# openai/iaf

Measured on AMD Instinct MI355X. Metric: IAF-step samples/sec (down_iaf2_nl posterior stack, forward + log-det), higher is better.
Workload: dtype f32 (operands split into 2 fp16 planes hi + lo 2^-11, 3 part-products on the fp16 MFMA in two fp32 accumulators: fp32-grade error, operands up to 65504)

## Files before the change

### iaf_amd/csrc/iaf_step_fused.hpp

```cpp
#pragma once
#include "iaf_conv_bf3.hpp"
#include "iaf_step_fused_types.hpp"
#ifndef IAF_HELPER_PRIO
#define IAF_HELPER_PRIO 0
#endif

#ifndef IAF_EXP_HOUT
#define IAF_EXP_HOUT 1
#endif
#ifndef IAF_EXP_HOUT8
#define IAF_EXP_HOUT8 1
#endif
template <int NHT, int NZT, int DEPTH, int W, int R, int XCH = 0, int PAIR = 0, int F16 = 0>
struct StepGeom {
    static constexpr int NZ = 16 * NZT, NH = 16 * NHT;
    static constexpr int NPL = F16 ? 2 : 3;
    static constexpr int RS = W + 2;
    static constexpr int Z8 = NZ / 8, Z16 = NPL * Z8 + 2;
    static constexpr int H8 = NH / 8, H16 = NPL * H8 + 2;
    static constexpr int RZ = XCH ? R + 1 : R + DEPTH + 1;
    static constexpr int rows_h(int l) { return XCH ? R : R + DEPTH - l; }
    static constexpr int rows_reg(int l) { return XCH ? R + 1 : R + DEPTH - l; }
    static constexpr int ZREG = 0;
    static constexpr int HREG0 = ZREG + RZ * RS * Z16;
// ... 250 lines not shown
    constexpr int CPX = G::CPX, CSTR = G::CSTR, CG = CPX / 4, NCIT = NH * CG, NCI = (NCIT + 255) / 256;
    f32x4 cv[NCI], cv2[NCI];
    unsigned cvalid = 0;
    auto load_ctx = [&]() {
        const int vpx = (H - r0) * W < CPX ? (H - r0) * W : CPX;
        constexpr bool REG = (256 % CG == 0) && (NCIT % 256 == 0);
        unsigned gi0 = 0, gstep = 0;
        bool in0 = true;
        if constexpr (REG) {
            const int c = tid / CG, g4 = (tid - c * CG) * 4;
            in0 = g4 < vpx;
            const int g4c = in0 ? g4 : 0;
            const int row = g4c / W, col4 = g4c - row * W;
            gi0 = 4u * (unsigned)(c * HW + gpix(r0 + row, col4 + (FLIP ? 3 : 0)));
            gstep = 4u * (unsigned)((256 / CG) * HW);
        }
        auto ctx_off = [&](int u, bool& inside) -> unsigned {
            if constexpr (REG) { inside = in0; return gi0 + (unsigned)u * gstep; }
            const int idx = tid + u * 256;
            const int ic = idx < NCIT ? idx : NCIT - 1;
            const int c = ic / CG, g4 = (ic - c * CG) * 4;
            inside = g4 < vpx;
            const int g4c = inside ? g4 : 0;
            const int row = g4c / W, col4 = g4c - row * W;
            return 4u * (unsigned)(c * HW + gpix(r0 + row, col4 + (FLIP ? 3 : 0)));
        };
#pragma unroll
        for (int u = 0; u < NCI; ++u) {
            bool inside;
            const unsigned gi = ctx_off(u, inside);
            cv[u] = ldf4(p.ctx + img_h, gi);
            cvalid |= (inside ? 1u : 0u) << u;
        }
        if (p.ctx2) {
#pragma unroll
            for (int u = 0; u < NCI; ++u) {
                bool inside;
                const unsigned gi = ctx_off(u, inside);
                cv2[u] = ldf4(p.ctx2 + img_h, gi);
            }
        }
    };
    auto zero_cols = [&]() {
        constexpr int ZROWS = RZ, H0ROWS = G::rows_reg(0), H1ROWS = 0;
        for (int i = tid; i < ZROWS * 2 * Z16; i += 256) {
            const int rs = i / Z16, u = i - rs * Z16;
            smem4[G::ZREG + ((rs >> 1) * RS + (rs & 1) * (W + 1)) * Z16 + u] = f32x4{0.f, 0.f, 0.f, 0.f};
        }
        for (int i = tid; i < (H0ROWS + H1ROWS) * 2 * H16; i += 256) {
            const int rs = i / H16, u = i - rs * H16;
            const int row = rs >> 1;
            const int base = row < H0ROWS ? G::HREG0 + row * RS * H16 : G::HREG1 + (row - H0ROWS) * RS * H16;
            smem4[base + (rs & 1) * (W + 1) * H16 + u] = f32x4{0.f, 0.f, 0.f, 0.f};
        }
    };
    auto stage_z = [&]() {
#pragma unroll
        for (int u = 0; u < ZU; ++u) {
            const int idx = tid + u * 256;
            if (idx < NIT) {
                const int q = idx / NPX, px = idx - q * NPX;
                const int row = px / W, col = px - row * W;
                f32x4 v = zv[u];
                if (!p.z) {
#pragma unroll
                    for (int r = 0; r < 4; ++r)
                        v[r] = (zv[u][r] + zq[0][u][r]) + __expf(0.5f * (2.f * (zq[1][u][r] + zq[2][u][r]))) * zq[3][u][r];
                }
                if (r0 + row >= H) v = f32x4{0.f, 0.f, 0.f, 0.f};
                split_store4(smem + (size_t)G::ZREG * 16, row * RS + col + 1, q, v, Z16, Z8);
            }
        }
    };

    constexpr unsigned XNLST = IAF_XCTL_LISTS;
    unsigned xcc = 0, xdead = 0;
    unsigned long long xdone = 0, xlists_done = 0;
    [[maybe_unused]] unsigned xmine = 0, xmine_n = 0;
    int xslot = 0;
    int half = 0;
    [[maybe_unused]] unsigned long long xt0 = 0;
    [[maybe_unused]] unsigned xlist = 0, xnl = 1;
    unsigned* xmail = (unsigned*)(smem + (size_t)G::CTX_OFF * 16);
    auto xch_take_begin = [&]() {
        if constexpr (TKT) {
            if (tid == 0) {
                asm volatile("s_getreg_b32 %0, hwreg(HW_REG_XCC_ID, 0, 4)" : "=s"(xcc));
                xcc &= 7u;
                xlist = xcc & (XNLST - 1u);
                if (p.xknob & 1u) xlist = (blockIdx.x * 2654435761u >> 13) & (XNLST - 1u);
                xnl = (unsigned)p.B < XNLST ? (unsigned)p.B : XNLST;
                if (xnl < XNLST) xlist %= xnl;
                if (p.xknob & 2u)
                    for (unsigned i = 0, n = (blockIdx.x * 40503u >> 4) & 63u; i < n; ++i) __builtin_amdgcn_s_sleep(64);
                xt0 = __hip_atomic_fetch_add(p.xctl + 32 * xlist, 1ull, __ATOMIC_RELAXED, XSCOPE);
                xdead = (unsigned)__hip_atomic_load(p.xctl + IAF_XCTL_STICKY, __ATOMIC_RELAXED, XSCOPE);
            }
        }
    };
    auto xch_take_finish = [&]() {
        if constexpr (TKT) {
            if (tid == 0) {
                unsigned long long v = xt0;
                unsigned y = xlist, t = 0, ny = 0;
                bool found = false;
                for (unsigned k = 0; k < xnl; ++k) {
                    if (k) { y = (xlist + k) % xnl; v = __hip_atomic_fetch_add(p.xctl + 32 * y, 1ull, __ATOMIC_RELAXED, XSCOPE); }
                    ny = (int)y < p.B ? (PAIR ? 2u : 1u) * (unsigned)p.nrb * (unsigned)((p.B - (int)y + (int)XNLST - 1) / (int)XNLST) : 0u;
                    t = (unsigned)v;
                    if (t < ny) { found = true; break; }
                }
                xmine = y; xmine_n = found ? ny : 0u;
                if (found) xdone = __hip_atomic_fetch_add(p.xctl + 32 * y + 16, 1ull, __ATOMIC_RELAXED, XSCOPE);
                unsigned ib = 0, ir = (unsigned)p.nrb - 1;
                const unsigned ti = PAIR ? t >> 1 : t;
                if (found) { ib = y + XNLST * (ti / (unsigned)p.nrb); ir = (unsigned)p.nrb - 1u - ti % (unsigned)p.nrb; }
                else xdead |= 2u;
                xmail[0] = ib; xmail[1] = ir; xmail[2] = xdead; xmail[3] = t & 1u;
                if (p.dbg) p.dbg[(size_t)blockIdx.x * 32 + 30] = 1ull + (((unsigned long long)y << 32) | t);
            }
            __syncthreads();
            b = __builtin_amdgcn_readfirstlane((int)xmail[0]);
            rbk = __builtin_amdgcn_readfirstlane((int)xmail[1]);
            xdead = __builtin_amdgcn_readfirstlane(xmail[2]);
            if constexpr (PAIR) half = __builtin_amdgcn_readfirstlane((int)xmail[3]);
            r0 = rbk * R;
            img_z = (size_t)b * NZ * HW; img_h = (size_t)b * NH * HW;
            xslot = b * p.nrb + rbk;
            if (xdead && tid == 0) {
                if (p.xerr) __hip_atomic_store(p.xerr, 0x100u | xdead, __ATOMIC_RELAXED, __HIP_MEMORY_SCOPE_SYSTEM);
                __hip_atomic_store(p.xctl + IAF_XCTL_STICKY, (unsigned long long)xdead, __ATOMIC_RELAXED, XSCOPE);
            }
        }
    };
    auto xch_next_epoch_a = [&]() {
        if constexpr (TKT) {
            if (tid == 0 && xmine_n && (unsigned)xdone == xmine_n - 1u)
                xlists_done = __hip_atomic_fetch_add(p.xctl + IAF_XCTL_DONE, 1ull, __ATOMIC_RELAXED, XSCOPE) + 1ull;
        }
    };
    auto xch_next_epoch_b = [&]() {
        if constexpr (TKT) {
            if (tid == 0 && (unsigned)xlists_done == (unsigned)(p.B < (int)XNLST ? p.B : (int)XNLST)) {
                for (int y = 0; y < (int)XNLST; ++y) {
                    __hip_atomic_store(p.xctl + 32 * y, 0ull, __ATOMIC_RELAXED, XSCOPE);
                    __hip_atomic_store(p.xctl + 32 * y + 16, 0ull, __ATOMIC_RELAXED, XSCOPE);
                }
                __hip_atomic_store(p.xctl + IAF_XCTL_DONE, 0ull, __ATOMIC_RELAXED, XSCOPE);
            }
        }
    };

    if constexpr (TKT) {
        xch_take_begin();
        if (!is_helper) {
            preload_w0();
            zero_cols();
        }
        xch_take_finish();
        if (!is_helper) {
            load_z();
            __builtin_amdgcn_sched_barrier(0);
            IAF_FSTAMP(8);
            stage_z();
        }
    } else if (!is_helper) {
        load_z();
        __builtin_amdgcn_sched_barrier(0);
        preload_w0();
        __builtin_amdgcn_sched_barrier(0);
        if constexpr (!HELP) load_ctx();
        __builtin_amdgcn_sched_barrier(0);
        IAF_FSTAMP(8);
        zero_cols();
        stage_z();
    }
    IAF_FSTAMP(9);
    __syncthreads();
    IAF_FSTAMP(1);
    auto store_ctx = [&]() {
        float* creg = (float*)(smem + (size_t)G::CTX_OFF * 16);
#pragma unroll
        for (int u = 0; u < NCI; ++u) {
            const int idx = tid + u * 256;
            if (NCIT % 256 == 0 || idx < NCIT) {
                const int c = idx / CG, g4 = (idx - c * CG) * 4;
                constexpr bool fl = FLIP;
                f32x4 v = cv[u];
                if (p.ctx2) v += cv2[u];
                if (!((cvalid >> u) & 1u)) v = f32x4{0.f, 0.f, 0.f, 0.f};
                *(f32x4*)(creg + c * CSTR + g4) = f32x4{fl ? v[3] : v[0], fl ? v[2] : v[1], fl ? v[1] : v[2], fl ? v[0] : v[3]};
            }
        }
    };

    int qbase = 0;
    auto conv_phase = [&](auto rd_c, auto npt_c, auto ntw_c, auto rows_c, auto emask_c, int in_reg, int in_s16, int in_c8, const f32x4* wbase,
                          int ncot, const int* tiles, f32x4 (*wr)[decltype(ntw_c)::value][3],
                          f32x4 (*acc_out)[decltype(ntw_c)::value], auto part_c, auto grp_c, auto accum_c, int pair0) __attribute__((always_inline)) {
        typedef decltype(part_c) P;
        constexpr int NPT = decltype(npt_c)::value, NTW = decltype(ntw_c)::value, ROWS = decltype(rows_c)::value;
        constexpr bool TRI = P::TAIL != 0;
        constexpr int nstep = P::NSTEP, s0 = 0;
        constexpr int EMASK = decltype(emask_c)::value;
        constexpr int LALLV = (EMASK == 0 && NTW > 1) ? ((1 << (NTW - 1)) - 1) : -1;
        constexpr std::integral_constant<int, LALLV> LALL{};
        constexpr int RD = decltype(rd_c)::value, U = RD + 1;
        constexpr int GRP = decltype(grp_c)::value;
        constexpr bool TALL = GRP >= 300 && GRP < 400, PTRI = GRP >= 100 && GRP < 300, HCMP = GRP >= 400;
        constexpr int PSG = F16 ? (NTW >= 2 ? 2 : 3) : TALL ? 1 : fused_acc_groups(HCMP ? NTWH : NTW);
        f32x4 acc[PSG][NPT][NTW];
        int xb[NPT];
#pragma unroll
        for (int q = 0; q < NPT; ++q) {
            int pix = (q + qbase) * 16 + pl;
            pix = pix < ROWS * W ? pix : ROWS * W - 1;
            const int row = pix / W, col = pix - row * W;
            xb[q] = in_reg + (row * RS + col + 1) * in_s16 + kk;
#pragma unroll
            for (int g = 0; g < PSG; ++g)
#pragma unroll
                for (int j = 0; j < NTW; ++j) acc[g][q][j] = f32x4{0.f, 0.f, 0.f, 0.f};
        }
        auto xaddr = [&](auto q_c, int s) __attribute__((always_inline)) -> int {
            int pair, tap;
            P::at(s < nstep ? s : nstep - 1, pair, tap);
// ... 164 lines not shown
                        const int pix = (q + qbase) * 16 + pl;
                        const int row = pix / W, col = pix - row * W;
                        if (pix < ROWS * W && row < R && r0 + row < H && (!save_half || (htile[j] >= NHT / 2) == (half != 0)))
                            *(f32x4*)(hsave + ((size_t)b * HW + (size_t)gpix(r0 + row, col)) * NH + htile[j] * 16 + 4 * kk) = vout[j][q];
                    }
                });
            }
            return;
        }
#pragma unroll
        for (int oi = 0; oi < NTWH * NPT; ++oi) {
            const int j = oi / NPT, q = oi % NPT;
            if (htile[j] >= NHT) continue;
            const f32x4 bi = bias[j];
            {
                if (j == NTWH - 1 && !((EMASK >> q) & 1)) continue;
                const int pix = (q + qbase) * 16 + pl;
                if (pix >= ROWS * W) continue;
                const int row = pix / W, col = pix - row * W;
                f32x4 v = acc[q][j] + bi;
                if constexpr (BORDER) { if (r0 + row < H) v += border_terms(bt, NH, htile[j] * 16 + 4 * kk, r0 + row, col); }
                if constexpr (WITH_CTX) v += cxv[q][j];
#pragma unroll
                for (int r = 0; r < 4; ++r) v[r] = elu_f(v[r]);
                if (r0 + row >= H) v = f32x4{0.f, 0.f, 0.f, 0.f};
                split_store4(smem + (size_t)out_reg * 16, row * RS + col + 1, htile[j] * 4 + kk, v, H16, H8);
                if (hsave && row < R && r0 + row < H && (!save_half || (htile[j] >= NHT / 2) == (half != 0)))
                    *(f32x4*)(hsave + ((size_t)b * HW + (size_t)gpix(r0 + row, col)) * NH + htile[j] * 16 + 4 * kk) = v;
            }
        }
    };

    constexpr int NZF = PAIR ? NZ / 2 : NZ;
    constexpr int NEL = (NZF * R * W + 255) / 256;
    float fz[NEL], fq[NEL][6];
    float fb[NEL][2];
    auto load_final_operands = [&]() {
        const int fcb = PAIR ? half * NZF : 0;
#pragma unroll
        for (int e = 0; e < NEL; ++e) {
            const int idx = tid + e * 256;
            const int ic = idx < NZF * R * W ? idx : NZF * R * W - 1;
            const int c = fcb + ic / (R * W), pix = ic % (R * W);
            const int rr = r0 + pix / W < H ? r0 + pix / W : H - 1;
            const unsigned gi = 4u * (unsigned)(c * HW + gpix(rr, pix & (W - 1)));
            const int cm = (c >> 4) * 32 + (c & 15);
            fb[e][0] = p.bias[DEPTH][cm]; fb[e][1] = p.bias[DEPTH][cm + 16];
            fz[e] = 0.f;
            if (p.mode == MODE_IAF || p.mode == MODE_INVERSE) fz[e] = ldf(p.zin + img_z, gi);
            if (p.mode == MODE_POSTERIOR) {
                fq[e][0] = ldf(p.qm + img_z, gi) + ldf(p.rm + img_z, gi); fq[e][1] = ldf(p.ql + img_z, gi) + ldf(p.rl + img_z, gi);
                fq[e][2] = ldf(p.eps + img_z, gi); fq[e][3] = ldf(p.pm + img_z, gi); fq[e][4] = ldf(p.pl + img_z, gi);
            }
        }
    };
    constexpr unsigned XSENT = F16 ? IAF_XSENT_F16 : IAF_XSENT;
    constexpr unsigned XNAN = F16 ? 0x7e007e00u : 0x7fc07fc0u;
    constexpr int XSC1 = 16;
    constexpr int XNU = W * H16, XNL = (XNU + 255) / 256;
    auto xch_rsrc = [&](int l, int slot) -> __amdgpu_buffer_rsrc_t {
        const unsigned long long a = (unsigned long long)(p.xh + ((size_t)l * p.B * p.nrb + slot) * G::xrow_bytes());
        const unsigned lo = __builtin_amdgcn_readfirstlane((unsigned)a), hi = __builtin_amdgcn_readfirstlane((unsigned)(a >> 32));
        return __builtin_amdgcn_make_buffer_rsrc((void*)(((unsigned long long)hi << 32) | lo), 0, (int)G::xrow_bytes(), 0x00020000);
    };
    constexpr int XNLH = (XNU + 255) / 256;
    auto xch_export = [&](int l, int reg) {
        if constexpr (XCH) {
            if (rbk > 0 && !((p.xknob & 8u) && b == 0 && rbk == p.nrb - 1 && l == 0)) {
                const __amdgpu_buffer_rsrc_t r = xch_rsrc(l, xslot);
                const f32x4* src = smem4 + reg + H16;
                f32x4 t[XNLH];
#pragma unroll
                for (int u = 0; u < XNLH; ++u) { const int i = htid + 256 * u; t[u] = src[i < XNU ? i : XNU - 1]; }
#pragma unroll
                for (int u = 0; u < XNLH; ++u)
                    __builtin_amdgcn_raw_buffer_store_b128(__builtin_bit_cast(u32x4, t[u]), r, 16 * (htid + 256 * u), 0, XSC1);
                if (l == 0 && p.dbg && htid == 0) {
                    p.dbg[(size_t)blockIdx.x * 32 + 27] = __builtin_readcyclecounter();
                    p.dbg[(size_t)blockIdx.x * 32 + 26] = (unsigned long long)xslot + 1;
                }
            }
        }
    };
    auto xch_import = [&](int l, int reg) {
        if constexpr (XCH) {
            f32x4* dst = smem4 + reg + (R * RS + 1) * H16;
            if (r0 + R < H) {
                const __amdgpu_buffer_rsrc_t r = xch_rsrc(l, xslot + 1);
                u32x4 t[XNLH];
                unsigned pad = 0;
#pragma unroll
                for (int u = 0; u < XNLH; ++u) {
                    const int i = htid + 256 * u;
                    if (i >= XNU || (i % H16) >= NPL * H8) pad |= 1u << u;
                }
                const int tmo = (p.xknob & 8u) ? (1 << 10) : (1 << 20);
                int it = xdead ? tmo : 0;
                if (p.dbg && htid == 0) p.dbg[(size_t)blockIdx.x * 32 + (l == 0 ? 14 : 18)] = __builtin_readcyclecounter();
                while (it < tmo) {
                    bool ok = true;
#pragma unroll
                    for (int u = 0; u < XNLH; ++u) t[u] = __builtin_amdgcn_raw_buffer_load_b128(r, 16 * (htid + 256 * u), 0, XSC1);
#pragma unroll
                    for (int u = 0; u < XNLH; ++u)
                        ok = ok && (((pad >> u) & 1u) || (t[u][0] != XSENT && t[u][1] != XSENT && t[u][2] != XSENT && t[u][3] != XSENT));
                    if (__all(ok)) break;
                    __builtin_amdgcn_s_sleep(8);
                    ++it;
                }
                if (p.dbg && htid == 0) {
                    p.dbg[(size_t)blockIdx.x * 32 + (l == 0 ? 16 : 19)] = __builtin_readcyclecounter();
                    p.dbg[(size_t)blockIdx.x * 32 + (l == 0 ? 24 : 25)] = (unsigned long long)it + 1;
                    p.dbg[(size_t)blockIdx.x * 32 + 26] = (unsigned long long)xslot + 1;
                }
                if (it < tmo) {
#pragma unroll
                    for (int u = 0; u < XNLH; ++u)
                        __builtin_amdgcn_raw_buffer_store_b128(u32x4{XSENT, XSENT, XSENT, XSENT}, r, 16 * (htid + 256 * u), 0, XSC1);
                } else {
#pragma unroll
                    for (int u = 0; u < XNLH; ++u) t[u] = u32x4{XNAN, XNAN, XNAN, XNAN};
                    if (lane == 0 && !xdead) {
                        if (p.xerr) __hip_atomic_store(p.xerr, 1u, __ATOMIC_RELAXED, __HIP_MEMORY_SCOPE_SYSTEM);
                        __hip_atomic_store(p.xctl + IAF_XCTL_STICKY, 1ull, __ATOMIC_RELAXED, XSCOPE);
                    }
                }
#pragma unroll
                for (int u = 0; u < XNLH; ++u) { const int i = htid + 256 * u; if (i < XNU) dst[i] = __builtin_bit_cast(f32x4, t[u]); }
                if (p.dbg && htid == 0) p.dbg[(size_t)blockIdx.x * 32 + (l == 0 ? 17 : 20)] = __builtin_readcyclecounter();
            } else {
                for (int i = htid; i < XNU; i += 256) dst[i] = f32x4{0.f, 0.f, 0.f, 0.f};
            }
        }
    };
    constexpr int PNL = PAIR ? (G::PUNITS + 255) / 256 : 1;
    constexpr int LASTH = ((DEPTH - 1) & 1) ? G::HREG1 : G::HREG0;
    auto pair_rsrc = [&](int hf) -> __amdgpu_buffer_rsrc_t {
        const unsigned long long a = (unsigned long long)(p.xh + ((size_t)xslot * 2 + hf) * G::prow_bytes());
        const unsigned lo = __builtin_amdgcn_readfirstlane((unsigned)a), hi = __builtin_amdgcn_readfirstlane((unsigned)(a >> 32));
        return __builtin_amdgcn_make_buffer_rsrc((void*)(((unsigned long long)hi << 32) | lo), 0, (int)G::prow_bytes(), 0x00020000);
    };
    auto pair_lds = [&](int i, int hf) -> int {
        const int sl = i / G::PUS, rem = i - sl * G::PUS;
        const int pn = rem / (H8 / 2), u = rem - pn * (H8 / 2);
        const int row = sl / W, col = sl - row * W;
        return LASTH + (row * RS + col + 1) * H16 + pn * H8 + hf * (H8 / 2) + u;
    };
    auto pair_export = [&]() {
        if constexpr (PAIR) {
            const __amdgpu_buffer_rsrc_t r = pair_rsrc(half);
            u32x4 t[PNL];
#pragma unroll
            for (int u = 0; u < PNL; ++u) {
                const int i = htid + 256 * u;
                t[u] = __builtin_bit_cast(u32x4, smem4[pair_lds(i < G::PUNITS ? i : G::PUNITS - 1, half)]);
            }
#pragma unroll
            for (int u = 0; u < PNL; ++u)
                __builtin_amdgcn_raw_buffer_store_b128(t[u], r, 16 * (htid + 256 * u), 0, XSC1);
            if (p.dbg && htid == 0) p.dbg[(size_t)blockIdx.x * 32 + 27] = __builtin_readcyclecounter();
        }
    };
    auto pair_import = [&]() {
        if constexpr (PAIR) {
            const __amdgpu_buffer_rsrc_t r = pair_rsrc(half ^ 1);
            u32x4 t[PNL];
            unsigned pad = 0;
#pragma unroll
            for (int u = 0; u < PNL; ++u)
                if (htid + 256 * u >= G::PUNITS) pad |= 1u << u;
            const int tmo = (p.xknob & 8u) ? (1 << 10) : (1 << 20);
            int it = xdead ? tmo : 0;
            if (p.dbg && htid == 0) p.dbg[(size_t)blockIdx.x * 32 + 18] = __builtin_readcyclecounter();
            while (it < tmo) {
                bool ok = true;
#pragma unroll
                for (int u = 0; u < PNL; ++u) t[u] = __builtin_amdgcn_raw_buffer_load_b128(r, 16 * (htid + 256 * u), 0, XSC1);
#pragma unroll
                for (int u = 0; u < PNL; ++u)
                    ok = ok && (((pad >> u) & 1u) || (t[u][0] != XSENT && t[u][1] != XSENT && t[u][2] != XSENT && t[u][3] != XSENT));
                if (__all(ok)) break;
                __builtin_amdgcn_s_sleep(8);
                ++it;
            }
            if (p.dbg && htid == 0) {
                p.dbg[(size_t)blockIdx.x * 32 + 19] = __builtin_readcyclecounter();
                p.dbg[(size_t)blockIdx.x * 32 + 25] = (unsigned long long)it + 1;
                p.dbg[(size_t)blockIdx.x * 32 + 26] = (unsigned long long)(2 * xslot + half) + 1;
            }
            const bool taken = it < tmo;
            if (!taken) {
#pragma unroll
                for (int u = 0; u < PNL; ++u) t[u] = u32x4{XNAN, XNAN, XNAN, XNAN};
            }
#pragma unroll
            for (int u = 0; u < PNL; ++u) { const int i = htid + 256 * u; if (i < G::PUNITS) smem4[pair_lds(i, half ^ 1)] = __builtin_bit_cast(f32x4, t[u]); }
            asm volatile("s_waitcnt lgkmcnt(0)" ::: "memory");
            __builtin_amdgcn_s_barrier();
            if (p.dbg && htid == 0) p.dbg[(size_t)blockIdx.x * 32 + 20] = __builtin_readcyclecounter();
            if (taken) {
#pragma unroll
                for (int u = 0; u < PNL; ++u)
                    __builtin_amdgcn_raw_buffer_store_b128(u32x4{XSENT, XSENT, XSENT, XSENT}, r, 16 * (htid + 256 * u), 0, XSC1);
            } else if (lane == 0 && !xdead) {
                if (p.xerr) __hip_atomic_store(p.xerr, 1u, __ATOMIC_RELAXED, __HIP_MEMORY_SCOPE_SYSTEM);
                __hip_atomic_store(p.xctl + IAF_XCTL_STICKY, 1ull, __ATOMIC_RELAXED, XSCOPE);
            }
        }
    };
    if constexpr (HELP) {
        if (is_helper) {
            __builtin_amdgcn_s_setprio(IAF_HELPER_PRIO);
            {
                constexpr int NCIH = (NCIT + 255) / 256;
                float* creg = (float*)(smem + (size_t)G::CTX_OFF * 16);
                const int vpx = (H - r0) * W < CPX ? (H - r0) * W : CPX;
                constexpr int RDL0 = PartL0::NSTEP - 1;
                [[maybe_unused]] f32x4 accu0[1][1], biu0[1], wrl0[HL0 ? RDL0 + 1 : 1][1][3];
                [[maybe_unused]] int lt0[1] = {NW * NFULL + (wave - NW_COMPUTE) % (NX ? NX : 1)};
                [[maybe_unused]] int q0 = -1;
                if constexpr (HL0) {
                    static_for<GN>([&](auto g_c) {
                        constexpr int GI = decltype(g_c)::value;
                        constexpr int EM = fused_extra_mask(NPT0, GN, GI);
                        static_assert(fused_popcount(EM) <= 1, "HL0: one pixel tile per left-over unit");
                        if constexpr (EM != 0) {
                            if ((wave - NW_COMPUTE) / NX == GI) q0 = EM == 1 ? 0 : EM == 2 ? 1 : EM == 4 ? 2 : 3;
                        }
                    });
                }
                f32x4 v[NCIH], v2[NCIH];
                unsigned cval = 0;
#pragma unroll
                for (int u = 0; u < NCIH; ++u) {
                    const int idx = htid + 256 * u, ic = idx < NCIT ? idx : NCIT - 1;
                    const int c = ic / CG, g4 = (ic - c * CG) * 4;
                    const bool inside = g4 < vpx;
                    const int g4c = inside ? g4 : 0, row = g4c / W, col4 = g4c - row * W;
                    const unsigned gi = 4u * (unsigned)(c * HW + gpix(r0 + row, col4 + (FLIP ? 3 : 0)));
                    v[u] = ldf4(p.ctx + img_h, gi);
                    if (p.ctx2) v2[u] = ldf4(p.ctx2 + img_h, gi);
                    cval |= (inside ? 1u : 0u) << u;
                }
                if constexpr (HL0) {
                    if (q0 >= 0) {
                        static_for<RDL0>([&](auto i) {
                            ring_load(std::integral_constant<int, 0>{}, std::integral_constant<int, NPL>{}, wrl0[decltype(i)::value], wb0, NHT, lt0,
                                      PartL0{}, decltype(i)::value, std::integral_constant<int, -1>{}, 0);
                        });
                        load_bias(std::integral_constant<int, 1>{}, lt0, p.bias[0], biu0);
                        qbase = q0;
                        conv_phase(std::integral_constant<int, RDL0>{}, std::integral_constant<int, 1>{}, std::integral_constant<int, 1>{},
                                   std::integral_constant<int, G::rows_h(0)>{}, std::integral_constant<int, 1>{}, G::ZREG, Z16, Z8, wb0, NHT, lt0,
                                   wrl0, accu0, PartL0{}, std::integral_constant<int, 300>{}, std::integral_constant<bool, false>{}, 0);
                        qbase = 0;
                    }
                }
#pragma unroll
                for (int u = 0; u < NCIH; ++u) {
                    const int idx = htid + 256 * u;
                    if (idx < NCIT) {
                        const int c = idx / CG, g4 = (idx - c * CG) * 4;
                        f32x4 t = v[u];
                        if (p.ctx2) t += v2[u];
                        if (!((cval >> u) & 1u)) t = f32x4{0.f, 0.f, 0.f, 0.f};
                        *(f32x4*)(creg + c * CSTR + g4) = FLIP ? f32x4{t[3], t[2], t[1], t[0]} : t;
                    }
                }
                __syncthreads();
                if constexpr (HL0) {
                    if (q0 >= 0) {
                        qbase = q0;
                        hidden_epilogue(std::integral_constant<int, 1>{}, std::integral_constant<int, G::rows_h(0)>{}, std::integral_constant<int, 1>{},
                                        std::integral_constant<int, 1>{}, std::integral_constant<int, 1>{}, lt0, accu0, biu0, G::HREG0, p.hsave[0],
                                        p.border[0], false);
                        qbase = 0;
                    }
                }
            }
            __syncthreads();
            xch_export(0, G::HREG0);
            typedef PairPart<NH / 32, 1> PartO8H;
            constexpr int RDOH8 = 3;
            [[maybe_unused]] f32x4 wroh8[G::HOUT8 ? RDOH8 + 1 : 1][NTWO][3];
            [[maybe_unused]] int ot8[NTWO];
#pragma unroll
            for (int j = 0; j < NTWO; ++j) ot8[j] = (wave - NW_COMPUTE) * NTWO + j;
            static_for<DEPTH - 1>([&](auto lm_c) {
                constexpr int l = decltype(lm_c)::value + 1;
                constexpr int IN_REG = ((l - 1) & 1) ? G::HREG1 : G::HREG0, OUT_REG = (l & 1) ? G::HREG1 : G::HREG0;
                if constexpr (XCH) {
                    xch_import(l - 1, IN_REG);
                    __syncthreads();
                }
                if constexpr (HLEFT) {
                    const int hw = wave - NW_COMPUTE;
                    constexpr int NPTL = (G::rows_h(l) * W + 15) / 16;
                    static_for<GN>([&](auto g_c) {
                        constexpr int GI = decltype(g_c)::value;
                        constexpr int EM = fused_extra_mask(NPTL, GN, GI);
                        static_assert(fused_popcount(EM) <= 1, "HLEFT: one pixel tile per left-over unit");
                        if constexpr (EM != 0) {
                            if (hw / NX != GI) return;
                            int lt[1] = {NW * NFULL + hw % NX};
                            qbase = EM == 1 ? 0 : EM == 2 ? 1 : EM == 4 ? 2 : 3;
                            const f32x4* wbl = (const f32x4*)p.wp3[l];
                            constexpr int RDL = 6;
                            f32x4 wrl[RDL + 1][1][3], accu[1][1], biu[1];
                            static_for<RDL>([&](auto i) {
                                ring_load(std::integral_constant<int, 0>{}, std::integral_constant<int, NPL>{}, wrl[decltype(i)::value], wbl, NHT, lt,
                                          PartHid{}, decltype(i)::value, std::integral_constant<int, -1>{}, 0);
                            });
                            load_bias(std::integral_constant<int, 1>{}, lt, p.bias[l], biu);
                            conv_phase(std::integral_constant<int, RDL>{}, std::integral_constant<int, 1>{}, std::integral_constant<int, 1>{},
                                       std::integral_constant<int, G::rows_h(l)>{}, std::integral_constant<int, 1>{}, IN_REG, H16, H8, wbl, NHT, lt,
                                       wrl, accu, PartHid{}, std::integral_constant<int, 300>{}, std::integral_constant<bool, false>{}, 0);
                            hidden_epilogue(std::integral_constant<int, 1>{}, std::integral_constant<int, G::rows_h(l)>{},
                                            std::integral_constant<int, 1>{}, std::integral_constant<int, 0>{}, std::integral_constant<int, 1>{}, lt,
                                            accu, biu, OUT_REG, p.hsave[l], p.border[l], false);
                            qbase = 0;
                        }
                    });
                }
                if constexpr (G::HOUT8 && l == DEPTH - 1) {
                    static_for<RDOH8>([&](auto i) {
                        ring_load(std::integral_constant<int, 0>{}, std::integral_constant<int, NTWO * NPL>{}, wroh8[decltype(i)::value],
                                  (const f32x4*)p.wp3[DEPTH], 2 * NZT, ot8, PartO8H{}, decltype(i)::value, std::integral_constant<int, -1>{}, 0);
                    });
                }
                __syncthreads();
                xch_export(l, OUT_REG);
            });
            if constexpr (XCH) {
                constexpr int LAST_REG = ((DEPTH - 1) & 1) ? G::HREG1 : G::HREG0;
                xch_import(DEPTH - 1, LAST_REG);
                if constexpr (G::HOUT) {
                    constexpr int NPTO_ = (R * W + 15) / 16;
                    const int hw = wave - NW_COMPUTE;
                    int ot[NTWO];
#pragma unroll
                    for (int j = 0; j < NTWO; ++j) ot[j] = hw * NTWO + j;
                    typedef BelowPar<NH / 32, 1> PartOBH;
                    constexpr int RDOH = 3;
                    const f32x4* wboh = (const f32x4*)p.wp3[DEPTH];
                    f32x4 wroh[RDOH + 1][NTWO][3], accoh[NPTO_][NTWO];
                    static_for<RDOH>([&](auto i) {
                        ring_load(std::integral_constant<int, 0>{}, std::integral_constant<int, NTWO * NPL>{}, wroh[decltype(i)::value], wboh, 2 * NZT,
                                  ot, PartOBH{}, decltype(i)::value, std::integral_constant<int, -1>{}, 0);
                    });
                    __syncthreads();
                    conv_phase(std::integral_constant<int, RDOH>{}, std::integral_constant<int, NPTO_>{}, std::integral_constant<int, NTWO>{},
                               std::integral_constant<int, R>{}, std::integral_constant<int, (1 << NPTO_) - 1>{}, LAST_REG,
                               H16, H8, wboh, 2 * NZT, ot, wroh, accoh, PartOBH{}, std::integral_constant<int, 0>{},
                               std::integral_constant<bool, false>{}, 0);
                    float* part1 = (float*)(smem + (size_t)G::XB_OFF * 16) + R * W * G::XB_STRIDE;
#pragma unroll
                    for (int j = 0; j < NTWO; ++j)
#pragma unroll
                        for (int q = 0; q < NPTO_; ++q) {
                            const int pix = q * 16 + pl;
                            if (pix >= R * W) continue;
#pragma unroll
                            for (int r = 0; r < 4; ++r) part1[pix * G::XB_STRIDE + ot[j] * 16 + 4 * kk + r] = accoh[q][j][r];
                        }
                } else {
                    __syncthreads();
                }
            }
            if constexpr (PAIR) {
                if (!((p.xknob & 8u) && b == 0 && rbk == 0 && half == 1)) pair_export();
                pair_import();
            }
            if constexpr (G::HOUT8) {
                constexpr int NPTO_ = (R * W + 15) / 16, LAST_REG = ((DEPTH - 1) & 1) ? G::HREG1 : G::HREG0;
                const f32x4* wboh = (const f32x4*)p.wp3[DEPTH];
                f32x4 accoh[NPTO_][NTWO];
                conv_phase(std::integral_constant<int, RDOH8>{}, std::integral_constant<int, NPTO_>{}, std::integral_constant<int, NTWO>{},
                           std::integral_constant<int, R>{}, std::integral_constant<int, (1 << NPTO_) - 1>{}, LAST_REG,
                           H16, H8, wboh, 2 * NZT, ot8, wroh8, accoh, PartO8H{}, std::integral_constant<int, 0>{},
                           std::integral_constant<bool, false>{}, 0);
                float* part1 = (float*)(smem + (size_t)G::XB_OFF * 16) + R * W * G::XB_STRIDE;
#pragma unroll
                for (int j = 0; j < NTWO; ++j)
#pragma unroll
                    for (int q = 0; q < NPTO_; ++q) {
                        const int pix = q * 16 + pl;
                        if (pix >= R * W) continue;
#pragma unroll
                        for (int r = 0; r < 4; ++r) part1[pix * G::XB_STRIDE + ot8[j] * 16 + 4 * kk + r] = accoh[q][j][r];
                    }
            }
            raise_range();
            __syncthreads();
            if (p.fin_ctl && p.mode == MODE_POSTERIOR) {
                unsigned* fmail = (unsigned*)smem;
                __syncthreads();
                if (htid == 0) {
                    const unsigned g = blockIdx.x & 7u, ng = (gridDim.x - g + 7u) >> 3, ngroups = gridDim.x < 8u ? gridDim.x : 8u;
                    unsigned last = 0;
                    if ((unsigned)__hip_atomic_fetch_add(p.fin_ctl + 32 * g, 1ull, __ATOMIC_RELAXED, XSCOPE) == ng - 1u) {
                        __hip_atomic_store(p.fin_ctl + 32 * g, 0ull, __ATOMIC_RELAXED, XSCOPE);
                        if ((unsigned)__hip_atomic_fetch_add(p.fin_ctl + 256, 1ull, __ATOMIC_RELAXED, XSCOPE) == ngroups - 1u) {
                            __hip_atomic_store(p.fin_ctl + 256, 0ull, __ATOMIC_RELAXED, XSCOPE);
                            last = 1;
                        }
                    }
                    fmail[0] = last;
                }
                __syncthreads();
                if (!fmail[0]) return;
                float* S = (float*)smem + 64;
                {
                    const __amdgpu_buffer_rsrc_t r = __builtin_amdgcn_make_buffer_rsrc((void*)p.kl_part, 0, p.B * p.nrb * NZ * 4, 0x00020000);
                    constexpr int Z4 = NZ / 4;
                    for (int i = htid; i < p.B * Z4; i += 256) {
                        const int bb = i / Z4, c4 = i - bb * Z4;
                        f32x4 a = f32x4{0.f, 0.f, 0.f, 0.f};
                        for (int k0 = 0; k0 < p.nrb; k0 += 8) {
                            u32x4 v8[8];
#pragma unroll
                            for (int k = 0; k < 8; ++k) {
                                const int rr = k0 + k < p.nrb ? k0 + k : p.nrb - 1;
                                v8[k] = __builtin_amdgcn_raw_buffer_load_b128(r, 4 * ((bb * p.nrb + rr) * NZ + 4 * c4), 0, XSC1);
                            }
#pragma unroll
                            for (int k = 0; k < 8; ++k)
                                if (k0 + k < p.nrb) a += __builtin_bit_cast(f32x4, v8[k]);
                        }
                        *(f32x4*)(S + (size_t)bb * NZ + 4 * c4) = a;
                    }
                }
                __syncthreads();
                if (htid < 64) {
                    const int GR = p.B / p.fin_groups;
                    float fbv = 0.f;
                    for (int g = 0; g < p.fin_groups; ++g) {
                        float a = 0.f;
                        if (htid < NZ) {
                            const float* Sg = S + (size_t)g * GR * NZ;
                            float m = 0.f;
                            for (int bb = 0; bb < GR; ++bb) m += Sg[(size_t)bb * NZ + htid];
                            a = fmaxf(m / (float)GR, p.fin_kl_min);
                            if (p.fin_gate && p.fin_kl_min > 0.f) p.fin_gate[g * NZ + htid] = (m / (float)GR > p.fin_kl_min) ? 1.f : 0.f;
                        }
#pragma unroll
                        for (int o = 32; o > 0; o >>= 1) a += __shfl_down(a, o, 64);
                        const float fb = __shfl(a, 0, 64);
                        if (htid == g) fbv = fb;
                    }
                    for (int b0 = 0; b0 < p.B; b0 += 64) {
// ... 11 lines not shown
            return;
        }
    }

    typedef std::conditional_t<XCH != 0, std::conditional_t<VAR == 0, PartOwnTri, PartOwn>, PartHid> PartH1;
    constexpr bool HO8 = G::HOUT8 && HELP;
    constexpr bool XK2 = PAIR || G::HOUT || HO8;
    typedef std::conditional_t<XCH != 0, PartOwn, std::conditional_t<HO8, PairPart<NPAIR_H, 0>, PartFull>> PartO1;
    int otile[NTWO];
#pragma unroll
    for (int j = 0; j < NTWO; ++j) otile[j] = wave * NTWO + j;
    constexpr int NHTP = NHT / 2, NFULLP = NHTP / NW, NTWP = NFULLP + 1;
    int ptile[NTWP];
    f32x4 wrp[PAIR ? UB : 1][NTWP][3];
    if constexpr (PAIR) {
#pragma unroll
        for (int j = 0; j < NTWP; ++j)
            ptile[j] = NHTP * half + ((j < NFULLP) ? ((j & 1) ? NW * (j + 1) - 1 - wave : wave + NW * j) : NW * NFULLP);
    }
    const int opar = wave & 1;
    constexpr int NPO = (NH / 2) / 32, NPR = NPAIR_H - NPO;
    const int opair_own = half ? NPAIR_H - NPO : 0, opair_rest = half ? 0 : NPO;
    if constexpr (PAIR) otile[0] = NZT * half + (wave >> 1);
    f32x4 wr1[UB][NTWH][3];
    f32x4 wrh1[HLEFT ? UB : 1][NTW1][3];
    f32x4 wro[UO][NTWO][3];
    const f32x4* wbo = (const f32x4*)p.wp3[DEPTH];
    auto preload_out = [&]() __attribute__((always_inline)) {
        if constexpr (PAIR) {
            static_for<2>([&](auto par_c) {
                if (opar != decltype(par_c)::value) return;
                static_for<RDO>([&](auto i) {
                    ring_load(std::integral_constant<int, 0>{}, std::integral_constant<int, NTWO * NPL>{}, wro[decltype(i)::value], wbo, 2 * NZT,
                              otile, PairPart<NPO, decltype(par_c)::value>{}, decltype(i)::value, ALL, opair_own);
                });
            });
            return;
        }
        static_for<RDO>([&](auto i) {
            ring_load(std::integral_constant<int, 0>{}, std::integral_constant<int, NTWO * NPL>{}, wro[decltype(i)::value], wbo, 2 * NZT,
                      otile, PartO1{}, decltype(i)::value, ALL, 0);
        });
    };
    auto preload_after = [&](auto l_c) __attribute__((always_inline)) {
        constexpr int l = decltype(l_c)::value;
        if constexpr (PAIR && l + 1 < DEPTH) {
            const f32x4* wbn = (const f32x4*)p.wp3[l + 1];
            static_for<RDH>([&](auto i) {
                ring_load(std::integral_constant<int, 0>{}, std::integral_constant<int, NTWP * NPL>{}, wrp[decltype(i)::value], wbn, NHT, ptile,
                          PartHid{}, decltype(i)::value, ALL, 0);
            });
        } else if constexpr (l + 1 < DEPTH && HLEFT) {
            const f32x4* wbn = (const f32x4*)p.wp3[l + 1];
            static_for<RDH>([&](auto i) {
                ring_load(std::integral_constant<int, 0>{}, std::integral_constant<int, NTW1 * NPL>{}, wrh1[decltype(i)::value], wbn, NHT, htile,
                          PartH1{}, decltype(i)::value, ALL, 0);
            });
        } else if constexpr (l + 1 < DEPTH) {
            const f32x4* wbn = (const f32x4*)p.wp3[l + 1];
            static_for<RDH>([&](auto i) {
                ring_load(std::integral_constant<int, 0>{}, std::integral_constant<int, NTWH * NPL>{},
                          ((l + 1) & 1) ? wr1[decltype(i)::value] : wr0[decltype(i)::value], wbn, NHT, htile, PartH1{}, decltype(i)::value,
                          ALL, 0);
            });
        } else {
            preload_out();
        }
    };
    static_for<GN>([&](auto g_c) {
        constexpr int GI = decltype(g_c)::value;
        if (xg != GI) return;
        constexpr int EM0 = HL0 ? (1 << NPT0) - 1 : (NX == 0 || !XSPLIT) ? (1 << NPT0) - 1 : fused_extra_mask(NPT0, GN, GI);
        f32x4 acc0[NPT0][NTW0], bi0[NTW0];
        load_bias(std::integral_constant<int, NTW0>{}, htile, p.bias[0], bi0);
        if constexpr (HL0)
            conv_phase(std::integral_constant<int, RD0>{}, std::integral_constant<int, NPT0>{}, std::integral_constant<int, NTW0>{},
                       std::integral_constant<int, G::rows_h(0)>{}, std::integral_constant<int, EM0>{}, G::ZREG, Z16, Z8, wb0, NHT, htile,
                       wrh0, acc0, PartL0{}, std::integral_constant<int, 400 + GI>{}, SET, 0);
        else
            conv_phase(std::integral_constant<int, RD0>{}, std::integral_constant<int, NPT0>{}, std::integral_constant<int, NTW0>{},
                       std::integral_constant<int, G::rows_h(0)>{}, std::integral_constant<int, EM0>{}, G::ZREG, Z16, Z8, wb0, NHT, htile,
                       wr0, acc0, PartL0{}, g_c, SET, 0);
        IAF_FSTAMP(6);
        xch_next_epoch_a();
        if constexpr (!HELP) store_ctx();
        if constexpr (DEPTH == 1) load_final_operands();
        preload_after(std::integral_constant<int, 0>{});
        IAF_FSTAMP(10);
        __syncthreads();
        IAF_FSTAMP(11);
        hidden_epilogue(std::integral_constant<int, NPT0>{}, std::integral_constant<int, G::rows_h(0)>{},
                        std::integral_constant<int, EM0>{}, std::integral_constant<int, 1>{}, std::integral_constant<int, NTW0>{}, htile, acc0, bi0,
                        G::HREG0, p.hsave[0], p.border[0], PAIR != 0);
    });
    __syncthreads();
    IAF_FSTAMP(2);
    if constexpr (PAIR) {
        constexpr int l = 1, IN_REG = G::HREG0, OUT_REG = G::HREG1;
        {
            constexpr int H1ROWS = G::rows_reg(1);
            for (int i = tid; i < H1ROWS * 2 * H16; i += 256) {
                const int rs = i / H16, u = i - rs * H16;
                smem4[G::HREG1 + ((rs >> 1) * RS + (rs & 1) * (W + 1)) * H16 + u] = f32x4{0.f, 0.f, 0.f, 0.f};
            }
        }
        constexpr int NPTL = (G::rows_h(l) * W + 15) / 16;
        const f32x4* wbl = (const f32x4*)p.wp3[l];
        static_for<2 * NW>([&](auto g_c) {
            constexpr int GI = decltype(g_c)::value % NW, HF = decltype(g_c)::value / NW;
            if (wave != GI || half != HF) return;
            constexpr int EML = fused_extra_mask(NPTL, NW, GI);
            f32x4 accl[NPTL][NTWP], bil[NTWP];
            load_bias(std::integral_constant<int, NTWP>{}, ptile, p.bias[l], bil);
            conv_phase(std::integral_constant<int, RDH>{}, std::integral_constant<int, NPTL>{}, std::integral_constant<int, NTWP>{},
                       std::integral_constant<int, G::rows_h(l)>{}, std::integral_constant<int, EML>{}, IN_REG, H16, H8, wbl, NHT, ptile,
                       wrp, accl, PartHid{}, std::integral_constant<int, 100 * (1 + HF) + GI>{}, SET, 0);
            IAF_FSTAMP(7);
            load_final_operands();
            preload_out();
            hidden_epilogue(std::integral_constant<int, NPTL>{}, std::integral_constant<int, G::rows_h(l)>{},
                            std::integral_constant<int, EML>{}, std::integral_constant<int, 0>{}, std::integral_constant<int, NTWP>{}, ptile, accl,
                            bil, OUT_REG, p.hsave[l], p.border[l], false);
            IAF_FSTAMP(12);
        });
        __syncthreads();
    }
    if constexpr (HLEFT) {
        constexpr int l = 1, IN_REG = G::HREG0, OUT_REG = G::HREG1;
        {
            constexpr int H1ROWS = G::rows_reg(1);
            for (int i = tid; i < H1ROWS * 2 * H16; i += 256) {
                const int rs = i / H16, u = i - rs * H16;
                smem4[G::HREG1 + ((rs >> 1) * RS + (rs & 1) * (W + 1)) * H16 + u] = f32x4{0.f, 0.f, 0.f, 0.f};
            }
        }
        constexpr int NPTL = (G::rows_h(l) * W + 15) / 16, EALL = (1 << NPTL) - 1;
        static_for<GN>([&](auto g_c) {
            constexpr int GI = decltype(g_c)::value;
            if (xg != GI) return;
            f32x4 accl[NPTL][NTW1], bil[NTW1];
            load_bias(std::integral_constant<int, NTW1>{}, htile, p.bias[l], bil);
            const f32x4* wbl = (const f32x4*)p.wp3[l];
            conv_phase(std::integral_constant<int, RDH>{}, std::integral_constant<int, NPTL>{}, std::integral_constant<int, NTW1>{},
                       std::integral_constant<int, G::rows_h(l)>{}, std::integral_constant<int, EALL>{}, IN_REG, H16, H8, wbl, NHT, htile,
                       wrh1, accl, PartH1{}, std::integral_constant<int, 400 + GI>{}, SET, 0);
            if constexpr (XCH) {
                static_for<RDH>([&](auto i) {
                    ring_load(std::integral_constant<int, 0>{}, std::integral_constant<int, NTW1 * NPL>{}, wrh1[decltype(i)::value], wbl, NHT, htile,
                              PartBelow{}, decltype(i)::value, ALL, 0);
                });
                IAF_FSTAMP(28);
                __syncthreads();
                IAF_FSTAMP(15);
                conv_phase(std::integral_constant<int, RDH>{}, std::integral_constant<int, NPTL>{}, std::integral_constant<int, NTW1>{},
                           std::integral_constant<int, G::rows_h(l)>{}, std::integral_constant<int, EALL>{}, IN_REG, H16, H8, wbl, NHT, htile,
                           wrh1, accl, PartBelow{}, std::integral_constant<int, 400 + GI>{}, ADD, 0);
            }
            IAF_FSTAMP(7);
            load_final_operands();
            preload_after(std::integral_constant<int, l>{});
            hidden_epilogue(std::integral_constant<int, NPTL>{}, std::integral_constant<int, G::rows_h(l)>{},
                            std::integral_constant<int, EALL>{}, std::integral_constant<int, 0>{}, std::integral_constant<int, NTW1>{}, htile, accl,
                            bil, OUT_REG, p.hsave[l], p.border[l], false);
            IAF_FSTAMP(12);
        });
        __syncthreads();
    }
    static_for<(PAIR || HLEFT) ? 0 : DEPTH - 1>([&](auto lm_c) {
        constexpr int l = decltype(lm_c)::value + 1;
        constexpr int IN_REG = ((l - 1) & 1) ? G::HREG1 : G::HREG0, OUT_REG = (l & 1) ? G::HREG1 : G::HREG0;
        if constexpr (l == 1) {
            constexpr int H1ROWS = G::rows_reg(1);
            for (int i = tid; i < H1ROWS * 2 * H16; i += 256) {
                const int rs = i / H16, u = i - rs * H16;
                smem4[G::HREG1 + ((rs >> 1) * RS + (rs & 1) * (W + 1)) * H16 + u] = f32x4{0.f, 0.f, 0.f, 0.f};
            }
        }
        constexpr int NPTL = (G::rows_h(l) * W + 15) / 16;
        static_for<GN>([&](auto g_c) {
            constexpr int GI = decltype(g_c)::value;
            if (xg != GI) return;
            constexpr int EML = (NX == 0 || !XSPLIT) ? (1 << NPTL) - 1 : fused_extra_mask(NPTL, GN, GI);
            f32x4 accl[NPTL][NTWH], bil[NTWH];
            load_bias(std::integral_constant<int, NTWH>{}, htile, p.bias[l], bil);
                const f32x4* wbl = (const f32x4*)p.wp3[l];
            conv_phase(std::integral_constant<int, RDH>{}, std::integral_constant<int, NPTL>{}, std::integral_constant<int, NTWH>{},
                       std::integral_constant<int, G::rows_h(l)>{}, std::integral_constant<int, EML>{}, IN_REG, H16, H8, wbl, NHT, htile,
                       (l & 1) ? wr1 : wr0, accl, PartH1{}, g_c, SET, 0);
            if constexpr (XCH) {
                static_for<RDH>([&](auto i) {
                    ring_load(std::integral_constant<int, 0>{}, std::integral_constant<int, NTWH * NPL>{},
                              (l & 1) ? wr1[decltype(i)::value] : wr0[decltype(i)::value], wbl, NHT, htile, PartBelow{}, decltype(i)::value, ALL, 0);
                });
                if constexpr (l == 1) IAF_FSTAMP(28);
                __syncthreads();
                if constexpr (l == 1) IAF_FSTAMP(15);
                conv_phase(std::integral_constant<int, RDH>{}, std::integral_constant<int, NPTL>{}, std::integral_constant<int, NTWH>{},
                           std::integral_constant<int, G::rows_h(l)>{}, std::integral_constant<int, EML>{}, IN_REG, H16, H8, wbl, NHT, htile,
                           (l & 1) ? wr1 : wr0, accl, PartBelow{}, g_c, ADD, 0);
            }
            if constexpr (l == 1) IAF_FSTAMP(7);
            if constexpr (l == DEPTH - 1) load_final_operands();
                preload_after(std::integral_constant<int, l>{});
            hidden_epilogue(std::integral_constant<int, NPTL>{}, std::integral_constant<int, G::rows_h(l)>{},
                            std::integral_constant<int, EML>{}, std::integral_constant<int, 0>{}, std::integral_constant<int, NTWH>{}, htile, accl,
                            bil, OUT_REG, p.hsave[l], p.border[l], false);
            if constexpr (l == 1) IAF_FSTAMP(12);
        });
        __syncthreads();
    });
    IAF_FSTAMP(3);
    raise_range();

    float* xbuf = (float*)(smem + (size_t)G::XB_OFF * 16);
    xch_next_epoch_b();
    if constexpr (PAIR) {
        f32x4 acco[NPTO][NTWO];
        constexpr int LAST_REG = ((DEPTH - 1) & 1) ? G::HREG1 : G::HREG0;
        static_for<2>([&](auto par_c) {
            constexpr int PAR = decltype(par_c)::value;
            if (opar != PAR) return;
            conv_phase(std::integral_constant<int, RDO>{}, std::integral_constant<int, NPTO>{}, std::integral_constant<int, NTWO>{},
                       std::integral_constant<int, R>{}, std::integral_constant<int, (1 << NPTO) - 1>{}, LAST_REG,
                       H16, H8, wbo, 2 * NZT, otile, wro, acco, PairPart<NPO, PAR>{}, std::integral_constant<int, 0>{}, SET, opair_own);
            static_for<RDO>([&](auto i) {
                ring_load(std::integral_constant<int, 0>{}, std::integral_constant<int, NTWO * NPL>{}, wro[decltype(i)::value], wbo, 2 * NZT,
                          otile, PairPart<NPR, PAR>{}, decltype(i)::value, ALL, opair_rest);
            });
            IAF_FSTAMP(29);
            __syncthreads();
            IAF_FSTAMP(21);
            conv_phase(std::integral_constant<int, RDO>{}, std::integral_constant<int, NPTO>{}, std::integral_constant<int, NTWO>{},
                       std::integral_constant<int, R>{}, std::integral_constant<int, (1 << NPTO) - 1>{}, LAST_REG,
                       H16, H8, wbo, 2 * NZT, otile, wro, acco, PairPart<NPR, PAR>{}, std::integral_constant<int, 0>{}, ADD, opair_rest);
        });
        IAF_FSTAMP(4);
        float* mine = xbuf + opar * (R * W * G::XB_STRIDE);
#pragma unroll
        for (int q = 0; q < NPTO; ++q) {
            const int pix = q * 16 + pl;
            if (pix >= R * W) continue;
#pragma unroll
            for (int r = 0; r < 4; ++r) mine[pix * G::XB_STRIDE + otile[0] * 16 + 4 * kk + r] = acco[q][0][r];
        }
    } else {
        f32x4 acco[NPTO][NTWO];
        constexpr int LAST_REG = ((DEPTH - 1) & 1) ? G::HREG1 : G::HREG0;
        conv_phase(std::integral_constant<int, RDO>{}, std::integral_constant<int, NPTO>{}, std::integral_constant<int, NTWO>{},
                   std::integral_constant<int, R>{}, std::integral_constant<int, (1 << NPTO) - 1>{}, LAST_REG,
                   H16, H8, wbo, 2 * NZT, otile, wro, acco, PartO1{}, std::integral_constant<int, 0>{}, SET, 0);
        if constexpr (XCH) {
            typedef std::conditional_t<G::HOUT, BelowPar<NPAIR_H, 0>, PartBelow> PartOB;
            static_for<RDO>([&](auto i) {
                ring_load(std::integral_constant<int, 0>{}, std::integral_constant<int, NTWO * NPL>{}, wro[decltype(i)::value], wbo, 2 * NZT,
                          otile, PartOB{}, decltype(i)::value, ALL, 0);
            });
            IAF_FSTAMP(29);
            __syncthreads();
            IAF_FSTAMP(21);
            conv_phase(std::integral_constant<int, RDO>{}, std::integral_constant<int, NPTO>{}, std::integral_constant<int, NTWO>{},
                       std::integral_constant<int, R>{}, std::integral_constant<int, (1 << NPTO) - 1>{}, LAST_REG,
                       H16, H8, wbo, 2 * NZT, otile, wro, acco, PartOB{}, std::integral_constant<int, 0>{}, ADD, 0);
        }
        IAF_FSTAMP(4);
        float* mine = xbuf;
#pragma unroll
        for (int j = 0; j < NTWO; ++j)
#pragma unroll
            for (int q = 0; q < NPTO; ++q) {
                const int pix = q * 16 + pl;
                if (pix >= R * W) continue;
#pragma unroll
                for (int r = 0; r < 4; ++r) mine[pix * G::XB_STRIDE + otile[j] * 16 + 4 * kk + r] = acco[q][j][r];
            }
    }
    __syncthreads();
    IAF_FSTAMP(13);

    float klv[NEL];
#pragma unroll
    for (int e = 0; e < NEL; ++e) klv[e] = 0.f;
    const int fcb = PAIR ? half * NZF : 0;
    if constexpr (FLAT) {
        float mr[NEL], sr[NEL];
        unsigned gio[NEL];
        bool live[NEL];
#pragma unroll
        for (int e = 0; e < NEL; ++e) {
            const int idx = tid + e * 256;
            const int ic = idx < NZF * R * W ? idx : NZF * R * W - 1;
            const int c = fcb + ic / (R * W), pix = ic % (R * W);
            const int row = pix / W, col = pix - row * W;
            live[e] = idx < NZF * R * W && r0 + row < H;
            const int rr = r0 + row < H ? r0 + row : H - 1;
            gio[e] = 4u * (unsigned)(c * HW + gpix(rr, col));
            const int cm = (c >> 4) * 32 + (c & 15);
            float m_raw = fb[e][0], s_raw = fb[e][1];
            if constexpr (BORDER) {
// ... 160 lines not shown
```

Before: 99760.

## Move ticket bookkeeping to helper wave and defer sentinel rearm off critical path

The work-ticket atomics now run on a helper-wave thread instead of thread 0 of a compute wave, and the epoch bookkeeping calls move into the helper's layer loop. Halo imports now end in a lighter barrier that only waits on LDS traffic (lgkmcnt) instead of a full __syncthreads. Rewriting the exchange buffer with sentinels is deferred until after the next layer's compute and export. The aim is to keep global atomic latency and sentinel stores off the compute waves' critical path. The risk is in ordering: the sentinel rearm and epoch reset now run at new points relative to other blocks' exports.

```diff
diff --git a/iaf_amd/csrc/iaf_step_fused.hpp b/iaf_amd/csrc/iaf_step_fused.hpp
--- a/iaf_amd/csrc/iaf_step_fused.hpp
+++ b/iaf_amd/csrc/iaf_step_fused.hpp
@@ -356,9 +356,11 @@
     [[maybe_unused]] unsigned long long xt0 = 0;
     [[maybe_unused]] unsigned xlist = 0, xnl = 1;
     unsigned* xmail = (unsigned*)(smem + (size_t)G::CTX_OFF * 16);
+    constexpr int XTID = 64 * NW_COMPUTE;
+    static_assert(!TKT || HELP, "the ticket is a helper thread's");
     auto xch_take_begin = [&]() {
         if constexpr (TKT) {
-            if (tid == 0) {
+            if (tid == XTID) {
                 asm volatile("s_getreg_b32 %0, hwreg(HW_REG_XCC_ID, 0, 4)" : "=s"(xcc));
                 xcc &= 7u;
                 xlist = xcc & (XNLST - 1u);
@@ -374,7 +376,7 @@
     };
     auto xch_take_finish = [&]() {
         if constexpr (TKT) {
-            if (tid == 0) {
+            if (tid == XTID) {
                 unsigned long long v = xt0;
                 unsigned y = xlist, t = 0, ny = 0;
                 bool found = false;
@@ -401,7 +403,7 @@
             r0 = rbk * R;
             img_z = (size_t)b * NZ * HW; img_h = (size_t)b * NH * HW;
             xslot = b * p.nrb + rbk;
-            if (xdead && tid == 0) {
+            if (xdead && tid == XTID) {
                 if (p.xerr) __hip_atomic_store(p.xerr, 0x100u | xdead, __ATOMIC_RELAXED, __HIP_MEMORY_SCOPE_SYSTEM);
                 __hip_atomic_store(p.xctl + IAF_XCTL_STICKY, (unsigned long long)xdead, __ATOMIC_RELAXED, XSCOPE);
             }
@@ -409,13 +411,13 @@
     };
     auto xch_next_epoch_a = [&]() {
         if constexpr (TKT) {
-            if (tid == 0 && xmine_n && (unsigned)xdone == xmine_n - 1u)
+            if (tid == XTID && xmine_n && (unsigned)xdone == xmine_n - 1u)
                 xlists_done = __hip_atomic_fetch_add(p.xctl + IAF_XCTL_DONE, 1ull, __ATOMIC_RELAXED, XSCOPE) + 1ull;
         }
     };
     auto xch_next_epoch_b = [&]() {
         if constexpr (TKT) {
-            if (tid == 0 && (unsigned)xlists_done == (unsigned)(p.B < (int)XNLST ? p.B : (int)XNLST)) {
+            if (tid == XTID && (unsigned)xlists_done == (unsigned)(p.B < (int)XNLST ? p.B : (int)XNLST)) {
                 for (int y = 0; y < (int)XNLST; ++y) {
                     __hip_atomic_store(p.xctl + 32 * y, 0ull, __ATOMIC_RELAXED, XSCOPE);
                     __hip_atomic_store(p.xctl + 32 * y + 16, 0ull, __ATOMIC_RELAXED, XSCOPE);
@@ -746,7 +748,8 @@
             }
         }
     };
-    auto xch_import = [&](int l, int reg) {
+    auto xch_import = [&](int l, int reg) -> bool {
+        bool taken = false;
         if constexpr (XCH) {
             f32x4* dst = smem4 + reg + (R * RS + 1) * H16;
             if (r0 + R < H) {
@@ -762,13 +765,13 @@
                 int it = xdead ? tmo : 0;
                 if (p.dbg && htid == 0) p.dbg[(size_t)blockIdx.x * 32 + (l == 0 ? 14 : 18)] = __builtin_readcyclecounter();
                 while (it < tmo) {
-                    bool ok = true;
+                    unsigned ok = 1u;
 #pragma unroll
                     for (int u = 0; u < XNLH; ++u) t[u] = __builtin_amdgcn_raw_buffer_load_b128(r, 16 * (htid + 256 * u), 0, XSC1);
 #pragma unroll
                     for (int u = 0; u < XNLH; ++u)
-                        ok = ok && (((pad >> u) & 1u) || (t[u][0] != XSENT && t[u][1] != XSENT && t[u][2] != XSENT && t[u][3] != XSENT));
-                    if (__all(ok)) break;
+                        ok &= ((pad >> u) & 1u) | (unsigned)((t[u][0] != XSENT) & (t[u][1] != XSENT) & (t[u][2] != XSENT) & (t[u][3] != XSENT));
+                    if (__all(ok != 0u)) break;
                     __builtin_amdgcn_s_sleep(8);
                     ++it;
                 }
@@ -777,11 +780,8 @@
                     p.dbg[(size_t)blockIdx.x * 32 + (l == 0 ? 24 : 25)] = (unsigned long long)it + 1;
                     p.dbg[(size_t)blockIdx.x * 32 + 26] = (unsigned long long)xslot + 1;
                 }
-                if (it < tmo) {
-#pragma unroll
-                    for (int u = 0; u < XNLH; ++u)
-                        __builtin_amdgcn_raw_buffer_store_b128(u32x4{XSENT, XSENT, XSENT, XSENT}, r, 16 * (htid + 256 * u), 0, XSC1);
-                } else {
+                taken = it < tmo;
+                if (!taken) {
 #pragma unroll
                     for (int u = 0; u < XNLH; ++u) t[u] = u32x4{XNAN, XNAN, XNAN, XNAN};
                     if (lane == 0 && !xdead) {
@@ -794,6 +794,21 @@
                 if (p.dbg && htid == 0) p.dbg[(size_t)blockIdx.x * 32 + (l == 0 ? 17 : 20)] = __builtin_readcyclecounter();
             } else {
                 for (int i = htid; i < XNU; i += 256) dst[i] = f32x4{0.f, 0.f, 0.f, 0.f};
+            }
+        }
+        return taken;
+    };
+    auto xch_handover = [&]() {
+        asm volatile("s_waitcnt lgkmcnt(0)" ::: "memory");
+        __builtin_amdgcn_s_barrier();
+    };
+    auto xch_rearm = [&](int l, bool taken) {
+        if constexpr (XCH) {
+            if (taken) {
+                const __amdgpu_buffer_rsrc_t r = xch_rsrc(l, xslot + 1);
+#pragma unroll
+                for (int u = 0; u < XNLH; ++u)
+                    __builtin_amdgcn_raw_buffer_store_b128(u32x4{XSENT, XSENT, XSENT, XSENT}, r, 16 * (htid + 256 * u), 0, XSC1);
             }
         }
     };
@@ -931,6 +946,7 @@
                         *(f32x4*)(creg + c * CSTR + g4) = FLIP ? f32x4{t[3], t[2], t[1], t[0]} : t;
                     }
                 }
+                xch_next_epoch_a();
                 __syncthreads();
                 if constexpr (HL0) {
                     if (q0 >= 0) {
@@ -953,10 +969,12 @@
             static_for<DEPTH - 1>([&](auto lm_c) {
                 constexpr int l = decltype(lm_c)::value + 1;
                 constexpr int IN_REG = ((l - 1) & 1) ? G::HREG1 : G::HREG0, OUT_REG = (l & 1) ? G::HREG1 : G::HREG0;
+                [[maybe_unused]] bool xtaken = false;
                 if constexpr (XCH) {
-                    xch_import(l - 1, IN_REG);
-                    __syncthreads();
-                }
+                    xtaken = xch_import(l - 1, IN_REG);
+                    xch_handover();
+                }
+                if constexpr (l == 1) xch_next_epoch_b();
                 if constexpr (HLEFT) {
                     const int hw = wave - NW_COMPUTE;
                     constexpr int NPTL = (G::rows_h(l) * W + 15) / 16;
@@ -994,10 +1012,12 @@
                 }
                 __syncthreads();
                 xch_export(l, OUT_REG);
+                xch_rearm(l - 1, xtaken);
             });
+            if constexpr (DEPTH == 1) xch_next_epoch_b();
             if constexpr (XCH) {
                 constexpr int LAST_REG = ((DEPTH - 1) & 1) ? G::HREG1 : G::HREG0;
-                xch_import(DEPTH - 1, LAST_REG);
+                const bool xtaken = xch_import(DEPTH - 1, LAST_REG);
                 if constexpr (G::HOUT) {
                     constexpr int NPTO_ = (R * W + 15) / 16;
                     const int hw = wave - NW_COMPUTE;
@@ -1012,7 +1032,7 @@
                         ring_load(std::integral_constant<int, 0>{}, std::integral_constant<int, NTWO * NPL>{}, wroh[decltype(i)::value], wboh, 2 * NZT,
                                   ot, PartOBH{}, decltype(i)::value, std::integral_constant<int, -1>{}, 0);
                     });
-                    __syncthreads();
+                    xch_handover();
                     conv_phase(std::integral_constant<int, RDOH>{}, std::integral_constant<int, NPTO_>{}, std::integral_constant<int, NTWO>{},
                                std::integral_constant<int, R>{}, std::integral_constant<int, (1 << NPTO_) - 1>{}, LAST_REG,
                                H16, H8, wboh, 2 * NZT, ot, wroh, accoh, PartOBH{}, std::integral_constant<int, 0>{},
@@ -1028,8 +1048,9 @@
                             for (int r = 0; r < 4; ++r) part1[pix * G::XB_STRIDE + ot[j] * 16 + 4 * kk + r] = accoh[q][j][r];
                         }
                 } else {
-                    __syncthreads();
-                }
+                    xch_handover();
+                }
+                xch_rearm(DEPTH - 1, xtaken);
             }
             if constexpr (PAIR) {
                 if (!((p.xknob & 8u) && b == 0 && rbk == 0 && half == 1)) pair_export();
@@ -1207,7 +1228,6 @@
                        std::integral_constant<int, G::rows_h(0)>{}, std::integral_constant<int, EM0>{}, G::ZREG, Z16, Z8, wb0, NHT, htile,
                        wr0, acc0, PartL0{}, g_c, SET, 0);
         IAF_FSTAMP(6);
-        xch_next_epoch_a();
         if constexpr (!HELP) store_ctx();
         if constexpr (DEPTH == 1) load_final_operands();
         preload_after(std::integral_constant<int, 0>{});
@@ -1338,7 +1358,6 @@
     raise_range();
 
     float* xbuf = (float*)(smem + (size_t)G::XB_OFF * 16);
-    xch_next_epoch_b();
     if constexpr (PAIR) {
         f32x4 acco[NPTO][NTWO];
         constexpr int LAST_REG = ((DEPTH - 1) & 1) ? G::HREG1 : G::HREG0;
```

New measurement: 102,600, median of 6. 1.03x the previous value.
